# danisotelo/qm_door

Hardware: AMD Instinct MI355X
Metric: MPC+WBC cycles/sec (AlienGo+Z1, N=100) (higher is better)
Workload: dtype f64; 1 GPU; configs[1]: batch=256 MPC instances per GPU, horizon N=100, dt=0.015, trot, 1 SQP iteration + filter line search + 3-level WBC; batch_per_gpu=256, global_batch=256, horizon_nodes=100, gait=trot, seed=0, collective=none

## Files before the change

qm_door_amd/csrc/kernels/aux_kernels.h:

```cpp
#pragma once
#include "layout.h"
#include "lq_kernel.h"

namespace qmk {

__global__ void __launch_bounds__(64) input_weight_kernel(const ProblemR* P, const real* zeros, real* Rw) {
  __shared__ real J[12 * 12];
  __shared__ real RJ[12 * 12];
  const int lane = threadIdx.x;
  const ModelR& md = P->model;
  const int dd = lane < AD_DIRS ? lane : AD_DIRS - 1;
  const AdIn in{P->settings.initial_state, zeros, P->settings.initial_state, dd, 0.0_r};
  FlowOut<Du, Du3, Du3> f;
  BaseMotion2<Du, Du3> bm;
  centroidalSweep2<Du, Du3, Du3>(
      md, P->settings.gravity, in,
      [&](int c, Vec3<Du>, Vec3<Du3> v) {
        if (lane >= 3 && lane < 15) { const int j = lane - 3; J[(3 * c + 0) * 12 + j] = v.x.e; J[(3 * c + 1) * 12 + j] = v.y.e; J[(3 * c + 2) * 12 + j] = v.z.e; }
      },
      [&](Vec3<Du>, const Mat3<Du>&) { return Vec3<Du3>(); }, f, bm);
  __syncthreads();
  const real* Rt = P->settings.R_task;
  for (int e = lane; e < 144; e += 64) {
    const int i = e / 12, j = e % 12;
// ... 92 lines not shown
  constexpr int NB = 4;
  const real* tg = gridP + size_t(inst) * (Np + 1);
  const int K = Np + 1, last = K - 1;
  for (int k0 = wave * NB; k0 <= Nn; k0 += nw * NB) {
    real t[NB]; int lb[NB];
#pragma unroll
    for (int q = 0; q < NB; ++q) { t[q] = gridN[size_t(inst) * (Nn + 1) + min(k0 + q, Nn)]; lb[q] = 0; }
    for (int base = 0; base < K; base += 64) {
      const int i = base + lane;
      const real g = tg[i < K ? i : 0];
#pragma unroll
      for (int q = 0; q < NB; ++q) lb[q] += qmPopCount(qmBallot(i < K && g < t[q]));
    }
    real ta[NB], tb[NB];
#pragma unroll
    for (int q = 0; q < NB; ++q) { const int ic = max(0, min(lb[q] - 1, K - 2)); ta[q] = tg[ic]; tb[q] = tg[min(ic + 1, last)]; }
    int idx[NB]; real alpha[NB];
#pragma unroll
    for (int q = 0; q < NB; ++q) {
      const int interval = lb[q] - 1;
      const real len = tb[q] - ta[q];
      const real a = (len > 2.0_r * REAL_EPS) ? (tb[q] - t[q]) / len : 1.0_r;
      const bool before = interval < 0 || K <= 1, after = !before && interval >= last;
      idx[q] = before ? 0 : (after ? max(last - 1, 0) : interval);
      alpha[q] = before ? 1.0_r : (after ? 0.0_r : a);
    }
    const bool isX = lane < 30, isU = lane >= 32 && lane < 62;
    const int c = isX ? lane : (isU ? lane - 32 : 0);
    real l[NB], r[NB];
#pragma unroll
    for (int q = 0; q < NB; ++q) {
      const int iu0 = min(idx[q], Np - 1), iu1 = min(idx[q] + 1, Np - 1);
      const real* pl = isU ? Up + (size_t(inst) * Np + iu0) * 30 : Xp + (size_t(inst) * (Np + 1) + idx[q]) * 30;
      const real* pr = isU ? Up + (size_t(inst) * Np + iu1) * 30 : Xp + (size_t(inst) * (Np + 1) + min(idx[q] + 1, last)) * 30;
      l[q] = pl[c]; r[q] = pr[c];
    }
    const real x0v = (x0 && isX) ? x0[size_t(inst) * 30 + c] : 0.0_r;
#pragma unroll
    for (int q = 0; q < NB; ++q) { QM_KEEP(l[q]); QM_KEEP(r[q]); }
#pragma unroll
    for (int q = 0; q < NB; ++q) {
      const int k = k0 + q;
      const real v = alpha[q] * l[q] + (1.0_r - alpha[q]) * r[q];
      if (k <= Nn && isX) warmX[(size_t(inst) * (Nn + 1) + k) * 30 + c] = (k == 0 && x0) ? x0v : v;
      else if (k < Nn && isU) warmU[(size_t(inst) * Nn + k) * 30 + c] = v;
    }
  }
}

__global__ void __launch_bounds__(64) policy_eval_kernel(int batch, int N, const real* tgrid, const real* X, const real* U, const int* modes, const real* tEval,
                                                         real* xOut, real* uOut, int* modeOut) {
  const int inst = blockIdx.x, lane = threadIdx.x;
  if (inst >= batch) return;
  const real* tg = tgrid + size_t(inst) * (N + 1);
  const real t = tEval[inst];
  int idx; real alpha;
  timeSegmentWave(tg, N + 1, t, lane, idx, alpha);
  const int kMode = gridCountBelow(tg + 1, N, t, lane);
  if (lane < 30) {
    const real* xl = X + (size_t(inst) * (N + 1) + idx) * 30;
    xOut[size_t(inst) * 30 + lane] = alpha * xl[lane] + (1.0_r - alpha) * xl[30 + lane];
  } else if (lane >= 32 && lane < 62) {
    const int i = lane - 32, iu0 = min(idx, N - 1), iu1 = min(idx + 1, N - 1);
    const real* ul = U + (size_t(inst) * N + iu0) * 30; const real* ur = U + (size_t(inst) * N + iu1) * 30;
    uOut[size_t(inst) * 30 + i] = alpha * ul[i] + (1.0_r - alpha) * ur[i];
  } else if (lane == 63) {
    modeOut[inst] = modes[size_t(inst) * (N + 1) + kMode];
  }
}

}
```

qm_door_amd/csrc/kernels/linesearch_kernel.h:

```cpp
#pragma once
#include "layout.h"
#include "ls_lds.h"
#include "schedule_dev.h"
#include "sweep_dev.h"

namespace qmk {

struct LsArgs {
  const ProblemR* P;
  const real* Rw;
  int batch, N, K, lineSearch;
  const real* eeContact;
  const real* tgrid; const real* dtgrid; const int* nodePhase;
  const real* X; const real* U; const real* dX; const real* dU;
  const real* targetTimes; const real* targetStates;
  const int* schedNum; const real* schedTimes; const int* schedModes;
  const real* metrics;
  const real* instStats;
  const int* nodeMode;
  real* Xt; real* Ut;
  real* outT; real* outX; real* outU; int* outMode; real* outStats;
  int iteration;
  int trialInLds;
  int* done;
};

inline int lsThreads(int B, int N, int cus) { return (B > cus && N + 1 <= LS_MAX_THREADS / 2) ? LS_MAX_THREADS / 2 : LS_MAX_THREADS; }
struct LsLaunch { int threads, dynamicLdsBytes, trialInLds; };
inline LsLaunch lsLaunch(int B, int N, int cus) {
  const int threads = lsThreads(B, N, cus), bytes = lsTrialLdsBytes(N, threads);
  return LsLaunch{threads, bytes, bytes > 0};
}

struct DblIn {
  const real* x; const real* u; real dtS; const real* k1;
  __device__ __forceinline__ real hn(int i) const { return x[i] + dtS * k1[i]; }
  __device__ __forceinline__ real euler(int i) const { return x[9 + i] + dtS * k1[9 + i]; }
  __device__ __forceinline__ real q(int j) const { return x[12 + j] + dtS * u[12 + j]; }
  __device__ __forceinline__ real qd(int j) const { return u[12 + j]; }
  __device__ __forceinline__ Vec3<real> force(int c) const { return Vec3<real>(u[3 * c], u[3 * c + 1], u[3 * c + 2]); }
};

template <class WP> __device__ __attribute__((noinline)) void nodePerformance(const ModelR& md, const SettingsR& st, WP Qw, WP Rw, int weightStructure, const real* bc, const Schedule& sched, const real* tTimes, const real* tStates, const real* contact, int K, real t, real dt, int phase,
                                       bool terminal, const real* x, const real* u, const real* xnext, real& cost, real& dyn, real& eq, real* xnOut = nullptr) {
  QM_TICK_DECL;
  const int mode = sched.modes[phase];
  real eePosRef[3], eeQuatRef[4];
  eeReference(tTimes, tStates, K, t, eePosRef, eeQuatRef);
  real Ke = 0.0_r, fRef[3] = {0.0_r, 0.0_r, 0.0_r}, pEnv[3] = {0.0_r, 0.0_r, 0.0_r};
  if (contact && !terminal) { Ke = st.ee_contact_stiffness; eeContactReference(tTimes, contact, K, t, fRef, pEnv); }
  real k1[12];
#pragma unroll
  for (int i = 0; i < 12; ++i) k1[i] = 0.0_r;
  real c = 0.0_r;
  dyn = 0.0_r; eq = 0.0_r;
  real phi[12];
#pragma unroll 1
  for (int stage = 0; stage < (terminal ? 1 : 2); ++stage) {
    const DblIn in{x, u, stage ? dt : 0.0_r, k1};
    Feet<real> feet;
    real f[12];
    BaseMotion<real> bm;
    centroidalSweep<real>(
        md, st.gravity, in, [&](int cc, Vec3<real> r, Vec3<real> v) { feet.set(cc, r, v); },
        [&](Vec3<real> r, const Mat3<real>& R) {
          const real sdt = stage ? dt : 0.0_r;
          const Vec3<real> fe(-Ke * (x[6] + sdt * k1[6] + r.x - pEnv[0]), -Ke * (x[7] + sdt * k1[7] + r.y - pEnv[1]), -Ke * (x[8] + sdt * k1[8] + r.z - pEnv[2]));
          if (stage == 0) {
            const real muF = Ke != 0.0_r ? st.ee_force_mu : 0.0_r;
            c += 0.5_r * muF * ((fe.x - fRef[0]) * (fe.x - fRef[0]) + (fe.y - fRef[1]) * (fe.y - fRef[1]) + (fe.z - fRef[2]) * (fe.z - fRef[2]));
            real qee[4];
            matrixToQuaternion(R, qee);
            const Vec3<real> od = quaternionDistance(qee, eeQuatRef);
            const real muP = terminal ? st.ee_final_mu_position : st.ee_mu_position, muO = terminal ? st.ee_final_mu_orientation : st.ee_mu_orientation;
            const real hx = x[6] + r.x - eePosRef[0], hy = x[7] + r.y - eePosRef[1], hz = x[8] + r.z - eePosRef[2];
            c += 0.5_r * muP * (hx * hx + hy * hy + hz * hz) + 0.5_r * muO * (od.x * od.x + od.y * od.y + od.z * od.z);
          }
// ... 227 lines not shown
        const real al = tr ? alpha * st.alpha_decay : alpha;
        if (tr && al < st.alpha_min) break;
        real s0 = 0, s1 = 0, s2 = 0;
        const int nTrial = N + 1 < half ? N + 1 : half;
        for (int i = tr * half; i < tr * half + nTrial; ++i) { s0 += red[0][i]; s1 += red[1][i]; s2 += red[2][i]; }
        m1 = s0; v1 = sqrt(s1 + s2);
        bool ok;
        if (!a.lineSearch) { ok = true; type = 0; }
        else if (v1 > st.g_max) { ok = v1 < (1.0_r - st.gamma_c) * viol0; type = 1; }
        else if (v1 < st.g_min && viol0 < st.g_min && al * armijo < 0.0_r) { ok = m1 < merit0 + st.armijo_factor * al * armijo; type = 3; }
        else { ok = m1 < merit0 - st.gamma_c * viol0 || v1 < (1.0_r - st.gamma_c) * viol0; type = 2; }
        accAlpha = al;
        if (ok) acc = 1.0_r;
      }
      ctl[LS_MERIT1] = m1; ctl[LS_VIOL1] = v1; ctl[LS_ACCEPTED] = acc; ctl[LS_STEP_TYPE] = real(type); ctl[LS_ALPHA] = accAlpha;
    }
    __syncthreads();
    QM_LS_CLOCK(4);
    merit1 = ctl[LS_MERIT1]; viol1 = ctl[LS_VIOL1]; stepType = int(ctl[LS_STEP_TYPE]);
    accepted = ctl[LS_ACCEPTED] != 0.0_r;
    const real lastAlpha = ctl[LS_ALPHA];
    __syncthreads();
    if (accepted) { alpha = lastAlpha; break; }
    alpha = lastAlpha * st.alpha_decay;
    if (alpha < st.alpha_min) break;
  }
  if (!accepted) { alpha = 0.0_r; stepType = 4; merit1 = merit0; viol1 = viol0; }
  real* oX = a.outX + size_t(inst) * (N + 1) * 30; real* oU = a.outU + size_t(inst) * N * 30;
  axpyStrided(oX, X, dX, alpha, (N + 1) * 30, tid, nthr);
  axpyStrided(oU, U, dU, alpha, N * 30, tid, nthr);
  for (int k = tid; k <= N; k += nthr) { a.outT[size_t(inst) * (N + 1) + k] = tg[k]; a.outMode[size_t(inst) * (N + 1) + k] = a.nodeMode[size_t(inst) * (N + 1) + k]; }
  QM_LS_CLOCK(5);
  const real sx = sumSquaresStrided(dX, (N + 1) * 30, tid, nthr), su = sumSquaresStrided(dU, N * 30, tid, nthr);
  __syncthreads();
  red[0][tid] = sx; red[1][tid] = su;
  __syncthreads();
  if (tid == 0) {
    real s0 = 0, s1 = 0;
    for (int i = 0; i < nthr; ++i) { s0 += red[0][i]; s1 += red[1][i]; }
    int conv = 0;
    if (a.iteration + 1 >= st.sqp_iterations) conv = 1;
    else if (alpha < st.alpha_min) conv = 2;
    else if (fabs(merit1 - merit0) < st.cost_tol && viol1 < st.g_min) conv = 3;
    else if (alpha * sqrt(s0) < st.delta_tol && alpha * sqrt(s1) < st.delta_tol) conv = 4;
    if (ricStatus != 0.0_r && conv == 0) conv = 2;
    a.done[inst] = conv;
    if (a.outStats) {
      real* s = a.outStats + size_t(inst) * QMGPU_NSTATS;
      s[0] = merit0; s[1] = viol0; s[2] = merit1; s[3] = viol1; s[4] = alpha; s[5] = real(stepType); s[6] = armijo; s[7] = ricStatus;
      s[8] = real(a.iteration + 1); s[9] = real(conv);
    }
  }
  QM_LS_CLOCK(6);
}
#endif

}
```

qm_door_amd/csrc/kernels/mpc_pipeline.h:

```cpp
#pragma once
#include <vector>

#include "../host/host_error.h"
#include "aux_kernels.h"
#include "ddp_kernel.h"
#include "gpu_rt.h"
#include "layout.h"
#include "linesearch_kernel.h"
#include "lq_kernel.h"
#include "riccati_kernel.h"

namespace qmk {

struct MpcBuffers {
  ProblemR* dP = nullptr;
  real *dRw = nullptr, *dZeros = nullptr;
  real *dTgrid = nullptr, *dDtgrid = nullptr, *dX = nullptr, *dU = nullptr, *dStages = nullptr, *dAdRows = nullptr, *dMetrics = nullptr, *dGains = nullptr, *ddX = nullptr, *ddU = nullptr;
  real *dXt = nullptr, *dUt = nullptr, *dInstStats = nullptr, *dDebug = nullptr;
  int *dStageNc = nullptr, *dNodeMode = nullptr, *dNodePhase = nullptr, *dDone = nullptr;
  real *dDdpX = nullptr, *dDdpU = nullptr, *dDdpMerit = nullptr;
  int cus = 256;
  size_t maxBatch = 0, maxNodes = 0;
};

struct MpcIo {
  int batch, N, K, lineSearch;
  double dtD;
  const double *t0D, *timeGridD, *schedTimesD;
  const real *x0, *targetTimes, *targetStates;
  const int* schedNum; const real* schedTimes; const int* schedModes;
  const real *warmX, *warmU;
  real *outT, *outX, *outU; int* outMode; real* outStats;
  const real* eeContact;
  int algorithm;
};

template <class Alloc> inline void allocateMpcBuffers(MpcBuffers& m, size_t B, size_t N, Alloc&& alloc) {
  const size_t N1 = N + 1;
  m.maxBatch = B; m.maxNodes = N;
  auto R = [&](size_t n, bool scratch = true) { return static_cast<real*>(alloc(n, sizeof(real), scratch)); };
  auto I = [&](size_t n) { return static_cast<int*>(alloc(n, sizeof(int), true)); };
  m.dP = static_cast<ProblemR*>(alloc(1, sizeof(ProblemR), false));
  m.dRw = R(QM_RW_DOUBLES, false);
  m.dZeros = R(64, false);
  m.dTgrid = R(B * N1);
  m.dDtgrid = R(B * N1);
  m.dNodePhase = I(B * N1);
  m.dX = R(B * N1 * 30);
  m.dU = R(B * N * 30);
  m.dStages = R(B * N1 * STAGE_DOUBLES);
  m.dAdRows = R(B * N1 * AD_DOUBLES);
  m.dMetrics = R(B * N1 * NODE_METRICS);
  m.dGains = R(B * N * GAIN_DOUBLES);
  m.ddX = R(B * N1 * 30);
  m.ddU = R(B * N * 30);
  m.dXt = R(2 * B * N1 * 30);
  m.dUt = R(2 * B * N * 30);
  m.dInstStats = R(B * 4);
  m.dStageNc = I(B * N1);
  m.dNodeMode = I(B * N1);
  m.dDone = I(B);
  int dev = 0, cus = 0;
  if (hipGetDevice(&dev) == hipSuccess && hipDeviceGetAttribute(&cus, hipDeviceAttributeMultiprocessorCount, dev) == hipSuccess && cus > 0) m.cus = cus;
}

template <class Alloc> inline void ensureDdpBuffers(MpcBuffers& m, Alloc&& alloc) {
  if (m.dDdpX) return;
  const size_t B = m.maxBatch, N = m.maxNodes;
  m.dDdpX = static_cast<real*>(alloc(size_t(DDP_MAX_TRIALS) * B * (N + 1) * 30, sizeof(real), true));
  m.dDdpU = static_cast<real*>(alloc(size_t(DDP_MAX_TRIALS) * B * N * 30, sizeof(real), true));
  m.dDdpMerit = static_cast<real*>(alloc(size_t(DDP_MAX_TRIALS) * B * 2, sizeof(real), true));
}

inline hipError_t prepareMpcKernels() {
  const hipError_t e = QM_ALLOW_DYNAMIC_LDS(riccati_kernel<RICCATI_WAVES>, RICCATI_LDS_BYTES);
  return e != hipSuccess ? e : QM_ALLOW_DYNAMIC_LDS(linesearch_kernel, QM_CU_LDS_BYTES - LS_STATIC_LDS_BYTES);
}

struct MpcStaging {
  real *x0 = nullptr, *targetTimes = nullptr, *targetStates = nullptr, *schedTimes = nullptr, *warmX = nullptr, *warmU = nullptr, *eeContact = nullptr;
};

template <class In> inline MpcIo makeMpcIo(const qmgpu_mpc_args& a, double dt, const MpcStaging& st, In&& in, real* outT, real* outX, real* outU, real* outStats) {
  const size_t B = size_t(a.batch), N = size_t(a.num_nodes), N1 = N + 1, K = size_t(a.num_target_knots);
  MpcIo io{};
  io.batch = a.batch; io.N = a.num_nodes; io.K = a.num_target_knots; io.lineSearch = a.line_search;
  io.dtD = dt; io.t0D = a.t0; io.timeGridD = a.time_grid; io.schedTimesD = a.sched_event_times;
  io.x0 = in(a.x0, st.x0, B * 30);
  io.targetTimes = in(a.target_times, st.targetTimes, B * K);
  io.targetStates = in(a.target_states, st.targetStates, B * K * QMGPU_NTARGET);
  io.schedNum = a.sched_num_events;
  io.schedTimes = in(a.sched_event_times, st.schedTimes, B * QMGPU_MAX_EVENTS);
  io.schedModes = a.sched_modes;
  io.warmX = in(a.warm_x, st.warmX, B * N1 * 30);
  io.warmU = in(a.warm_u, st.warmU, B * N * 30);
  io.eeContact = in(a.ee_contact_ref, st.eeContact, B * K * 6);
  io.outT = outT; io.outX = outX; io.outU = outU; io.outMode = a.out_mode; io.outStats = outStats;
  io.algorithm = a.algorithm;
  return io;
}

enum TimingEvent { EV_START, EV_AD_NODE, EV_LQ_NODE, EV_RICCATI, EV_LINE_SEARCH, EV_WBC_START, EV_WBC_END, TIMING_EVENTS = EV_WBC_END + 1 };
inline void recordTiming(hipEvent_t* ev, TimingEvent which, hipStream_t s) { if (ev) (void)hipEventRecord(ev[which], s); }

inline void enqueueLqRiccati(hipStream_t s, const MpcBuffers& m, const MpcIo& io, real* debug, hipEvent_t* ev) {
  const int B = io.batch, N = io.N;
  LqArgs la{m.dP, m.dRw, B, N, io.K, m.dTgrid, m.dDtgrid, m.dNodePhase, m.dX, m.dU, io.targetTimes, io.targetStates, io.schedNum, io.schedTimes,
            io.schedModes, m.dZeros, m.dStages, m.dStageNc, m.dNodeMode, m.dMetrics, debug, m.dAdRows, m.dDone, io.eeContact};
  QM_LAUNCH(ad_node_kernel, adGridFor(B * (N + 1)), 64, s, la);
  recordTiming(ev, EV_AD_NODE, s);
  QM_LAUNCH(lq_node_kernel, B * (N + 1), 64, s, la);
  recordTiming(ev, EV_LQ_NODE, s);
  RiccatiArgs ra{B, N, m.dStages, m.dStageNc, m.dDtgrid, io.x0, m.dX, m.dGains, m.ddX, m.ddU, m.dInstStats, m.dDone};
  QM_LAUNCH_DYN(riccati_kernel<RICCATI_WAVES>, B, RICCATI_WAVES * 64, RICCATI_LDS_BYTES, s, ra);
  recordTiming(ev, EV_RICCATI, s);
}

inline void enqueueMpcKernels(hipStream_t s, const MpcBuffers& m, const MpcIo& io, int iterations, bool debugLq, hipEvent_t* ev) {
  const int B = io.batch, N = io.N;
  recordTiming(ev, EV_START, s);
  for (int it = 0; it < iterations; ++it) {
    InitArgs ia{m.dP, B, N, io.dtD, io.t0D, io.timeGridD, io.schedTimesD, io.x0, it == 0 ? io.warmX : io.outX, it == 0 ? io.warmU : io.outU, io.schedNum, io.schedModes,
                m.dTgrid, m.dDtgrid, m.dNodePhase, m.dX, m.dU, it, m.dDone};
    QM_LAUNCH(mpc_init_kernel, B, 128, s, ia);
    enqueueLqRiccati(s, m, io, debugLq ? m.dDebug : nullptr, ev);
    const LsLaunch shape = lsLaunch(B, N, m.cus);
    LsArgs ls{m.dP, m.dRw, B, N, io.K, io.lineSearch, io.eeContact, m.dTgrid, m.dDtgrid, m.dNodePhase, m.dX, m.dU, m.ddX, m.ddU, io.targetTimes, io.targetStates, io.schedNum,
              io.schedTimes, io.schedModes, m.dMetrics, m.dInstStats, m.dNodeMode, m.dXt, m.dUt, io.outT, io.outX, io.outU, io.outMode, io.outStats, it, shape.trialInLds, m.dDone};
    QM_LAUNCH_DYN(linesearch_kernel, B, shape.threads, shape.dynamicLdsBytes, s, ls);
    recordTiming(ev, EV_LINE_SEARCH, s);
  }
}

inline void enqueueDdpKernels(hipStream_t s, const MpcBuffers& m, const MpcIo& io, int trials, hipEvent_t* ev) {
  const int B = io.batch, N = io.N;
  recordTiming(ev, EV_START, s);
  InitArgs ia{m.dP, B, N, io.dtD, io.t0D, io.timeGridD, io.schedTimesD, io.x0, io.warmX, io.warmU, io.schedNum, io.schedModes, m.dTgrid, m.dDtgrid, m.dNodePhase, m.dX, m.dU, 0, m.dDone};
  QM_LAUNCH(mpc_init_kernel, B, 128, s, ia);
  DdpArgs ra{m.dP, m.dRw, B, N, io.K, 0, io.eeContact, m.dTgrid, m.dDtgrid, m.dNodePhase, io.x0, m.dX, m.dU, io.targetTimes, io.targetStates, io.schedNum, io.schedTimes, io.schedModes,
             m.dStages, m.dStageNc, m.dGains, m.dX, m.dU, m.dDdpMerit};
  if (!io.warmX) QM_LAUNCH(ddp_rollout_kernel, (B + 63) / 64, 64, s, ra);
  enqueueLqRiccati(s, m, io, nullptr, ev);
  ra.trials = trials; ra.Xout = m.dDdpX; ra.Uout = m.dDdpU;
  QM_LAUNCH(ddp_rollout_kernel, (B * trials + 63) / 64, 64, s, ra);
  DdpSelectArgs sa{m.dP, B, N, trials, m.dTgrid, m.dNodeMode, m.dX, m.dU, m.dMetrics, m.dInstStats, m.dDdpX, m.dDdpU, m.dDdpMerit, io.outT, io.outX, io.outU, io.outMode, io.outStats, m.dDone};
  QM_LAUNCH(ddp_select_kernel, B, 256, s, sa);
  recordTiming(ev, EV_LINE_SEARCH, s);
}

inline int ddpTrialCount(double minStep, double maxStep) {
  int n = 0;
  for (double a = maxStep; a >= minStep && n < DDP_MAX_TRIALS; a *= 0.5) ++n;
  return n > 0 ? n : 1;
}

template <class Alloc> inline void enqueueMpcSolve(hipStream_t s, MpcBuffers& m, const MpcIo& io, const qmgpu_settings& settings, bool debugLq, hipEvent_t* ev, Alloc&& alloc) {
  if (io.algorithm != QMGPU_ALG_SQP && io.algorithm != QMGPU_ALG_DDP) throw std::invalid_argument("unknown qmgpu_mpc_args::algorithm");
  if (io.algorithm == QMGPU_ALG_DDP) {
    ensureDdpBuffers(m, alloc);
    enqueueDdpKernels(s, m, io, ddpTrialCount(settings.ddp_min_step, settings.ddp_max_step), ev);
  } else {
    enqueueMpcKernels(s, m, io, settings.sqp_iterations > 1 ? settings.sqp_iterations : 1, debugLq, ev);
  }
  HIP_CHECK(hipGetLastError());
}

}
```

qm_door_amd/csrc/kernels/schedule_dev.h:

```cpp
#pragma once
#include "problem_r.h"
#include "contact_rows.h"
#include "gpu_rt.h"

namespace qmk {

struct Schedule {
  int numEvents;
  const real* eventTimes;
  const int* modes;
};

__device__ __forceinline__ int nodePhaseAt(const Schedule& s, real t) {
  int i = 0;
  while (i < s.numEvents && s.eventTimes[i] <= t) ++i;
  return i;
}

__device__ __forceinline__ void cubic(real t0, real p0, real v0, real t1, real p1, real v1, real t, real& pos, real& vel) {
  const real dt = t1 - t0, dp = p1 - p0, dv = v1 - v0;
  const real c1 = v0 * dt, c2 = -(3.0_r * v0 + dv) * dt + 3.0_r * dp, c3 = (2.0_r * v0 + dv) * dt - 2.0_r * dp;
  const real tn = (t - t0) / dt;
  pos = ((c3 * tn + c2) * tn + c1) * tn + p0;
  vel = ((3.0_r * c3 * tn + 2.0_r * c2) * tn + c1) / dt;
// ... 1 lines not shown

__device__ inline void swingReference(const SettingsR& st, const Schedule& s, int leg, real t, int phase, real& zpos, real& zvel) {
  const int numPhases = s.numEvents + 1;
  int startIdx = -1;
  for (int ip = phase - 1; ip >= 0; --ip) if (contactOf(s.modes[ip], leg)) { startIdx = ip; break; }
  int finalIdx = numPhases - 1;
  for (int ip = phase + 1; ip < numPhases; ++ip) if (contactOf(s.modes[ip], leg)) { finalIdx = ip - 1; break; }
  const real tStart = (startIdx >= 0) ? s.eventTimes[startIdx] : ((s.numEvents > 0 ? s.eventTimes[0] : t) - st.touchdown_after_horizon);
  const real tFinal = (finalIdx < numPhases - 1) ? s.eventTimes[finalIdx] : ((s.numEvents > 0 ? s.eventTimes[s.numEvents - 1] : t) + st.touchdown_after_horizon);
  const real scaling = fmin(1.0_r, (tFinal - tStart) / st.swing_time_scale);
  const real tMid = 0.5_r * (tStart + tFinal), midHeight = scaling * st.swing_height;
  if (t < tMid) cubic(tStart, 0.0_r, scaling * st.liftoff_velocity, tMid, midHeight, 0.0_r, t, zpos, zvel);
  else cubic(tMid, midHeight, 0.0_r, tFinal, 0.0_r, scaling * st.touchdown_velocity, t, zpos, zvel);
}

__device__ __forceinline__ void timeSegment(const real* times, int K, real t, int& index, real& alpha) {
  if (K <= 1) { index = 0; alpha = 1.0_r; return; }
  int lb = 0;
  while (lb < K && times[lb] < t) ++lb;
  const int interval = lb - 1, last = K - 1;
  if (interval < 0) { index = 0; alpha = 1.0_r; }
  else if (interval >= last) { index = max(last - 1, 0); alpha = 0.0_r; }
  else {
    const real len = times[interval + 1] - times[interval];
    index = interval;
    alpha = (len > 2.0_r * REAL_EPS) ? (times[interval + 1] - t) / len : 1.0_r;
  }
}

__device__ __forceinline__ int gridCountBelow(const real* times, int K, real t, int lane) {
  int lb = 0;
  for (int base = 0; base < K; base += 64) {
    const int i = base + lane;
    const bool below = i < K && times[i < K ? i : 0] < t;
    const unsigned long long m = qmBallot(below);
    lb += qmPopCount(m);
    if (m != ~0ull) break;
  }
  return lb;
}
__device__ __forceinline__ void timeSegmentWave(const real* times, int K, real t, int lane, int& index, real& alpha) {
  if (K <= 1) { index = 0; alpha = 1.0_r; return; }
  const int lb = gridCountBelow(times, K, t, lane);
  const int interval = lb - 1, last = K - 1;
  if (interval < 0) { index = 0; alpha = 1.0_r; }
  else if (interval >= last) { index = max(last - 1, 0); alpha = 0.0_r; }
  else {
    const real len = times[interval + 1] - times[interval];
    index = interval;
    alpha = (len > 2.0_r * REAL_EPS) ? (times[interval + 1] - t) / len : 1.0_r;
  }
}

__device__ inline void eeReference(const real* times, const real* states, int K, real t, real pos[3], real quat[4]) {
  int idx; real alpha;
  timeSegment(times, K, t, idx, alpha);
  const real* lhs = states + size_t(idx) * QMGPU_NTARGET;
  if (K <= 1) {
    for (int i = 0; i < 3; ++i) pos[i] = lhs[30 + i];
    for (int i = 0; i < 4; ++i) quat[i] = lhs[33 + i];
    return;
  }
  const real* rhs = lhs + QMGPU_NTARGET;
  for (int i = 0; i < 3; ++i) pos[i] = alpha * lhs[30 + i] + (1.0_r - alpha) * rhs[30 + i];
  const real tt = 1.0_r - alpha;
  const real* a = lhs + 33; const real* b = rhs + 33;
  const real d = a[0] * b[0] + a[1] * b[1] + a[2] * b[2] + a[3] * b[3];
  const real absD = fabs(d);
  real s0, s1;
  if (absD >= 1.0_r - REAL_EPS) { s0 = 1.0_r - tt; s1 = tt; }
  else { const real theta = acos(absD), sinTheta = sin(theta); s0 = sin((1.0_r - tt) * theta) / sinTheta; s1 = sin(tt * theta) / sinTheta; }
  if (d < 0) s1 = -s1;
  for (int i = 0; i < 4; ++i) quat[i] = s0 * a[i] + s1 * b[i];
}
__device__ inline void eeContactReference(const real* times, const real* contact, int K, real t, real fref[3], real env[3]) {
  int idx; real alpha;
  timeSegment(times, K, t, idx, alpha);
  const real* lhs = contact + size_t(idx) * 6;
  const real* rhs = K > 1 ? lhs + 6 : lhs;
  for (int i = 0; i < 3; ++i) { fref[i] = alpha * lhs[i] + (1.0_r - alpha) * rhs[i]; env[i] = alpha * lhs[3 + i] + (1.0_r - alpha) * rhs[3 + i]; }
}
__device__ __forceinline__ real xReference(const real* states, int K, int idx, real alpha, int i) {
  const real* lhs = states + size_t(idx) * QMGPU_NTARGET;
  if (K <= 1) return lhs[i];
  return alpha * lhs[i] + (1.0_r - alpha) * lhs[QMGPU_NTARGET + i];
}

struct Barrier {
  real mu, delta;
  __device__ __forceinline__ real value(real h) const { const real q = (h - 2.0_r * delta) / delta; return h > delta ? -mu * log(h) : mu * (-log(delta) + 0.5_r * q * q - 0.5_r); }
  __device__ __forceinline__ real d1(real h) const { return h > delta ? -mu / h : mu * ((h - 2.0_r * delta) / (delta * delta)); }
  __device__ __forceinline__ real d2(real h) const { return h > delta ? mu / (h * h) : mu / (delta * delta); }
  __device__ __forceinline__ void eval(real h, real logDelta, real& val, real& g, real& hs) const {
    if (h > delta) { const real r = 1.0_r / h; val = -mu * log(h); g = -mu * r; hs = mu * r * r; }
    else { const real q = (h - 2.0_r * delta) / delta; val = mu * (-logDelta + 0.5_r * q * q - 0.5_r); g = mu * ((h - 2.0_r * delta) / (delta * delta)); hs = mu / (delta * delta); }
  }
  __device__ __forceinline__ real valueL(real h, real logDelta) const {
    if (h > delta) return -mu * log(h);
    const real q = (h - 2.0_r * delta) / delta;
    return mu * (-logDelta + 0.5_r * q * q - 0.5_r);
  }
};

}
```

qm_door_amd/csrc/qmgpu_api.hip:

```cpp
#include <algorithm>
#include <cstdio>
#include <cstring>
#include <memory>
#include <string>
#include <vector>

#include "../../include/qmgpu.h"
#include "host/host_error.h"
#include "kernels/mpc_pipeline.h"
#include "kernels/feedback_kernel.h"
#include "kernels/value_kernel.h"
#include "kernels/dual_kernel.h"
#include "kernels/wbc_kernel.h"
#include "kernels/frontend_kernel.h"
#include "mpc32.h"

using namespace qmhost;
using namespace qmk;

struct DeviceGuard {
  int prev = -1;
  explicit DeviceGuard(int device, bool mayThrow = true) {
    if (hipGetDevice(&prev) != hipSuccess) prev = -1;
    if (prev == device) { prev = -1; return; }
// ... 185 lines not shown
    double v;
    if (e < nx) v = X[size_t(inst) * nx + e];
    else if (e < nx + nu) v = U[size_t(inst) * nu + (e - nx)];
    else if (e < nx + nu + QMGPU_NWBC_OUT) v = wbc[size_t(inst) * QMGPU_NWBC_OUT + (e - nx - nu)];
    else v = double(modes[size_t(inst) * (N + 1) + (e - nx - nu - QMGPU_NWBC_OUT)]);
    row[e] = v;
  }
}

#ifdef QM_RICCATI_TIMING
int qmgpu_debug_riccati_ticks(unsigned long long* out64, int reset) {
  if (hipDeviceSynchronize() != hipSuccess) return QMGPU_ERR_HIP;
  if (out64 && hipMemcpyFromSymbol(out64, HIP_SYMBOL(qmk::qmRiccatiTicks), sizeof(unsigned long long) * 2048) != hipSuccess) return QMGPU_ERR_HIP;
  if (reset) { static unsigned long long z[2048] = {}; if (hipMemcpyToSymbol(HIP_SYMBOL(qmk::qmRiccatiTicks), z, sizeof(z)) != hipSuccess) return QMGPU_ERR_HIP; }
  return QMGPU_OK;
}
int qmgpu_debug_ad_wg_clocks(unsigned long long* out64, int count) {
  if (hipDeviceSynchronize() != hipSuccess) return QMGPU_ERR_HIP;
  if (count > 2 * QM_AD_WG_CLOCKS) count = 2 * QM_AD_WG_CLOCKS;
  if (hipMemcpyFromSymbol(out64, HIP_SYMBOL(qmk::qmAdWgClock), sizeof(unsigned long long) * size_t(count)) != hipSuccess) return QMGPU_ERR_HIP;
  return QMGPU_OK;
}
#endif

int qmgpu_debug_poison(qmgpu_handle h) {
  return onHandle(h, [&]() {
    joinWbc(h);
    for (auto& sc : h->scratch) HIP_CHECK(hipMemsetAsync(sc.first, 0xFF, sc.second, h->stream));
    constexpr int kDoubles = QM_CU_LDS_BYTES / 8;
    HIP_CHECK(QM_ALLOW_DYNAMIC_LDS(lds_poison_kernel, kDoubles * 8));
    QM_LAUNCH_DYN(lds_poison_kernel, 4096, 256, kDoubles * 8, h->stream, kDoubles, static_cast<double*>(nullptr));
    HIP_CHECK(hipGetLastError());
  });
}

int qmgpu_enable_debug(qmgpu_handle h, int enable) {
  return onHandle(h, [&]() {
    if (enable && h->dtype != QMGPU_F64) throw std::invalid_argument("the per-node LQ dump exists in the fp64 path only");
    if (enable && !h->m.dDebug) h->m.dDebug = h->alloc<double>(size_t(h->maxBatch) * (h->maxNodes + 1) * DBG_DOUBLES);
    h->debugLq = enable != 0;
  });
}

static void checkMpcArgs(qmgpu_handle h, const qmgpu_mpc_args* a) {
  if (!a) throw std::invalid_argument("null argument");
  if (a->batch < 1 || a->num_nodes < 1 || a->num_target_knots < 1) throw std::invalid_argument("batch, num_nodes and num_target_knots must be positive");
  if (a->batch > h->maxBatch || a->num_nodes > h->maxNodes) throw CapacityError("batch / num_nodes exceed the capacity given to qmgpu_create");
  if (h->dtype == QMGPU_F32 && a->num_target_knots > QMGPU_F32_MAX_TARGET_KNOTS) throw CapacityError("an fp32 handle stages at most QMGPU_F32_MAX_TARGET_KNOTS target knots per instance");
  if (!a->x0 || !a->target_times || !a->target_states || !a->sched_num_events || !a->sched_event_times || !a->sched_modes) throw std::invalid_argument("missing MPC input pointer");
  if (!a->time_grid && !a->t0) throw std::invalid_argument("either t0 or time_grid is required");
  if (!a->out_t || !a->out_x || !a->out_u || !a->out_mode) throw std::invalid_argument("missing MPC output pointer");
}

static void enqueueMpc(qmgpu_handle h, const qmgpu_mpc_args* a) {
  const qmgpu_settings& settings = h->hostProblem.settings;
  hipEvent_t* ev = h->timing ? h->ev : nullptr;
  if (h->dtype == QMGPU_F32) {
    qmk32::enqueue(h->m32, h->stream, a, settings, ev, h->rawAlloc);
  } else {
    const MpcIo io = makeMpcIo(*a, settings.dt, MpcStaging{}, [](const double* src, double*, size_t) { return src; }, a->out_t, a->out_x, a->out_u, a->out_stats);
    enqueueMpcSolve(h->stream, h->m, io, settings, h->debugLq, ev, h->rawAlloc);
  }
  h->lastBatch = a->batch; h->lastN = a->num_nodes; h->lastAlgorithm = a->algorithm;
  h->lastDebugLq = h->dtype == QMGPU_F64 && a->algorithm == QMGPU_ALG_SQP && h->debugLq;
}

static void enqueueWbc(qmgpu_handle h, const qmgpu_wbc_args* w, hipStream_t stream) {
  if (!w || w->batch < 1) throw std::invalid_argument("bad WBC arguments");
  if (w->batch > h->maxBatch) throw CapacityError("WBC batch exceeds the capacity given to qmgpu_create");
  if (!w->state_desired || !w->input_desired || !w->rbd_measured || !w->mode || !w->period || !w->time || !w->input_last || !w->out) throw std::invalid_argument("missing WBC pointer");
  static_assert(sizeof(unsigned long long) == sizeof(uint64_t), "working-set words");
  WbcArgs wa{h->m.dP, w->batch, w->variant, w->state_desired, w->input_desired, w->rbd_measured, w->mode, w->period, w->time, w->input_last, w->out, w->out_status, w->ee_force,
             reinterpret_cast<unsigned long long*>(w->working_set)};
  QM_LAUNCH_DYN(wbc_kernel, w->batch, WBC_THREADS, WBC_LDS_BYTES, stream, wa);
  HIP_CHECK(hipGetLastError());
}

static void beginTiming(qmgpu_handle h) {
  if (h->timing) h->ev = h->ring[h->callCount % qmgpu_context::kRing];
}
static void finishTiming(qmgpu_handle h, bool mpc, bool wbc) {
  if (!h->timing) return;
  h->ringKind[h->callCount % qmgpu_context::kRing] = (mpc ? 1 : 0) | (wbc ? 2 : 0);
  ++h->callCount;
}
static void readTiming(qmgpu_handle h, long call, double* ms6) {
  hipEvent_t* ev = h->ring[call % qmgpu_context::kRing];
  const int kind = h->ringKind[call % qmgpu_context::kRing];
  const bool mpc = kind & 1, wbc = kind & 2;
  const TimingEvent first = mpc ? EV_START : EV_WBC_START, last = wbc ? EV_WBC_END : EV_LINE_SEARCH;
  HIP_CHECK(hipEventSynchronize(ev[last]));
  auto elapsed = [&](TimingEvent from, TimingEvent to) { float ms = 0.f; HIP_CHECK(hipEventElapsedTime(&ms, ev[from], ev[to])); return double(ms); };
  for (int i = 0; i < 6; ++i) ms6[i] = 0.0;
  if (mpc) for (int k = EV_AD_NODE; k <= EV_LINE_SEARCH; ++k) ms6[k - EV_AD_NODE] = elapsed(TimingEvent(k - 1), TimingEvent(k));
  if (wbc) ms6[4] = elapsed(EV_WBC_START, EV_WBC_END);
  ms6[5] = elapsed(first, last);
}

int qmgpu_mpc_solve_batch(qmgpu_handle h, const qmgpu_mpc_args* args) {
  return onHandle(h, [&]() { checkMpcArgs(h, args); beginTiming(h); enqueueMpc(h, args); finishTiming(h, true, false); });
}

int qmgpu_policy_eval_batch(qmgpu_handle h, int batch, int num_nodes, const double* t_grid, const double* X, const double* U, const int32_t* modes, const double* t_eval,
                            double* x_out, double* u_out, int32_t* mode_out) {
  if (!t_grid || !X || !U || !modes || !t_eval || !x_out || !u_out || !mode_out || batch < 1 || num_nodes < 1) return setError(QMGPU_ERR_INVALID_ARGUMENT, "bad arguments");
  return onHandle(h, [&]() {
    QM_LAUNCH(policy_eval_kernel, batch, 64, h->stream, batch, num_nodes, t_grid, X, U, modes, t_eval, x_out, u_out, mode_out);
    HIP_CHECK(hipGetLastError());
  });
}

static void checkLastSqpSolve(qmgpu_handle h, int batch, int num_nodes, const char* what) {
  const std::string w(what);
  if (h->dtype != QMGPU_F64) throw std::invalid_argument(w + " exists for QMGPU_F64 handles only");
  if (h->lastBatch < 1) throw std::invalid_argument(w + " needs a solve on this handle first");
  if (h->lastAlgorithm != QMGPU_ALG_SQP) throw std::invalid_argument(w + " exists for QMGPU_ALG_SQP solves only");
  if (batch != h->lastBatch || num_nodes != h->lastN) throw std::invalid_argument("batch / num_nodes differ from the last solve on this handle");
}

int qmgpu_mpc_feedback_batch(qmgpu_handle h, int batch, int num_nodes, const double* X, const double* U, double* K, double* uff, int32_t* status) {
  if (!X || !U || !K || !uff || batch < 1 || num_nodes < 1) return setError(QMGPU_ERR_INVALID_ARGUMENT, "bad feedback arguments");
  return onHandle(h, [&]() {
    checkLastSqpSolve(h, batch, num_nodes, "the feedback policy");
    static_assert(sizeof(int) == sizeof(int32_t), "status words");
    FeedbackArgs fa{batch, num_nodes, h->m.dStages, h->m.dGains, h->m.dInstStats, X, U, K, uff, status};
    QM_LAUNCH(feedback_gain_kernel, batch * (num_nodes + 1), 64, h->stream, fa);
    HIP_CHECK(hipGetLastError());
  });
}

int qmgpu_mpc_value_function_batch(qmgpu_handle h, int batch, int num_nodes, double* Sm, double* Sv, double* sv_lin, double* x_lin, int32_t* status) {
  if (!Sm || !Sv || batch < 1 || num_nodes < 1) return setError(QMGPU_ERR_INVALID_ARGUMENT, "bad value-function arguments");
  return onHandle(h, [&]() {
    checkLastSqpSolve(h, batch, num_nodes, "the value function");
    ValueArgs va{batch, num_nodes, h->m.dStages, h->m.dGains, h->m.dDtgrid, h->m.dInstStats, h->m.dX, Sm, Sv, sv_lin, x_lin, status};
    QM_LAUNCH_DYN(value_function_kernel, batch, VALUE_THREADS, VALUE_LDS_BYTES, h->stream, va);
    HIP_CHECK(hipGetLastError());
  });
}

int qmgpu_mpc_dual_batch(qmgpu_handle h, int batch, int num_nodes, double* costate, double* nu, int32_t* nc, int32_t* status) {
  if (!costate || batch < 1 || num_nodes < 1) return setError(QMGPU_ERR_INVALID_ARGUMENT, "bad dual-solution arguments");
  return onHandle(h, [&]() {
    checkLastSqpSolve(h, batch, num_nodes, "the dual solution");
    if (nu && !(h->lastDebugLq && h->m.dDebug)) throw std::invalid_argument("nu needs the LQ dump of the solve: call qmgpu_enable_debug(h, 1) before it");
    static_assert(sizeof(int) == sizeof(int32_t), "nc and status words");
    DualArgs da{batch, num_nodes, h->m.dStages, h->m.dGains, h->m.dDtgrid, h->m.dInstStats, h->m.ddX, h->m.ddU, nu ? h->m.dDebug : nullptr, h->m.dStageNc, costate, nu, nc, status};
    QM_LAUNCH_DYN(costate_kernel, batch, DUAL_THREADS, DUAL_LDS_BYTES, h->stream, da);
// ... 23 lines not shown

int qmgpu_frontend_batch(qmgpu_handle h, const qmgpu_frontend_args* a) {
  if (!a || a->batch < 1 || !a->rbd_measured || !a->time || !a->command_kind || !a->command || !a->last_ee_target || !a->x0 || !a->target_times || !a->target_states)
    return setError(QMGPU_ERR_INVALID_ARGUMENT, "bad front-end arguments");
  return onHandle(h, [&]() {
    FrontendArgs fa{h->m.dP, *a};
    QM_LAUNCH(frontend_kernel, (a->batch + 63) / 64, 64, h->stream, fa);
    HIP_CHECK(hipGetLastError());
  });
}

int qmgpu_gait_schedule_batch(qmgpu_handle h, int batch, const qmgpu_gait* templates, int num_templates, const int32_t* gait_index, const int32_t* prev_mode,
                              const double* t_phase0, const double* t_begin, const double* t_end, int32_t* sched_num_events, double* sched_event_times, int32_t* sched_modes, int32_t* status) {
  if (batch < 1 || !templates || num_templates < 1 || num_templates > 64 || !gait_index || !t_phase0 || !t_begin || !t_end || !sched_num_events || !sched_event_times || !sched_modes)
    return setError(QMGPU_ERR_INVALID_ARGUMENT, "bad gait schedule arguments");
  return onHandle(h, [&]() {
    if (!h->dGaits) h->dGaits = h->alloc<qmgpu_gait>(64, false);
    HIP_CHECK(hipMemcpyAsync(h->dGaits, templates, sizeof(qmgpu_gait) * num_templates, hipMemcpyHostToDevice, h->stream));
    HIP_CHECK(hipStreamSynchronize(h->stream));
    GaitArgs ga{batch, num_templates, h->dGaits, gait_index, prev_mode, h->hostProblem.settings.phase_transition_stance_time, t_phase0, t_begin, t_end, sched_num_events, sched_event_times, sched_modes, status};
    QM_LAUNCH(gait_schedule_kernel, (batch + 63) / 64, 64, h->stream, ga);
    HIP_CHECK(hipGetLastError());
  });
}

int qmgpu_wbc_solve_batch(qmgpu_handle h, const qmgpu_wbc_args* args) {
  return onHandle(h, [&]() {
    joinWbc(h);
    beginTiming(h);
    if (h->timing) HIP_CHECK(hipEventRecord(h->ev[EV_WBC_START], h->stream));
    enqueueWbc(h, args, h->stream);
    if (h->timing) HIP_CHECK(hipEventRecord(h->ev[EV_WBC_END], h->stream));
    finishTiming(h, false, true);
  });
}

int qmgpu_warm_start_batch(qmgpu_handle h, int batch, int prev_nodes, const double* prev_grid, const double* prev_X, const double* prev_U, int new_nodes,
                           const double* new_grid, const double* x0, double* warm_x, double* warm_u) {
  if (!prev_grid || !prev_X || !prev_U || !new_grid || !warm_x || !warm_u || batch < 1 || prev_nodes < 1 || new_nodes < 1)
    return setError(QMGPU_ERR_INVALID_ARGUMENT, "bad warm-start arguments");
  if (warm_x == prev_X || warm_u == prev_U) return setError(QMGPU_ERR_INVALID_ARGUMENT, "warm-start outputs must not alias the previous solution");
  return onHandle(h, [&]() {
    QM_LAUNCH(warm_start_kernel, batch, 256, h->stream, batch, prev_nodes, prev_grid, prev_X, prev_U, new_nodes, new_grid, x0, warm_x, warm_u);
    HIP_CHECK(hipGetLastError());
  });
}

int qmgpu_cycle_batch(qmgpu_handle h, const qmgpu_mpc_args* mpc, const double* t_eval, qmgpu_wbc_args* wbc) {
  if (!t_eval || !wbc) return setError(QMGPU_ERR_INVALID_ARGUMENT, "null argument");
  return onHandle(h, [&]() {
    checkMpcArgs(h, mpc);
    if (wbc->batch != mpc->batch) throw std::invalid_argument("MPC and WBC batch sizes differ");
    beginTiming(h);
    enqueueMpc(h, mpc);
    joinWbc(h);
    QM_LAUNCH(policy_eval_kernel, mpc->batch, 64, h->stream, mpc->batch, mpc->num_nodes, mpc->out_t, mpc->out_x, mpc->out_u, mpc->out_mode, t_eval, h->dPolX, h->dPolU,
              h->dPolMode);
    qmgpu_wbc_args w = *wbc;
    w.state_desired = h->dPolX; w.input_desired = h->dPolU; w.mode = h->dPolMode;
    hipStream_t ws = h->stream;
    if (h->overlap) {
      HIP_CHECK(hipEventRecord(h->evPolicy, h->stream));
      HIP_CHECK(hipStreamWaitEvent(h->wbcStream, h->evPolicy, 0));
      ws = h->wbcStream;
    }
    if (h->timing) HIP_CHECK(hipEventRecord(h->ev[EV_WBC_START], ws));
    enqueueWbc(h, &w, ws);
    if (h->timing) HIP_CHECK(hipEventRecord(h->ev[EV_WBC_END], ws));
    if (h->overlap) { HIP_CHECK(hipEventRecord(h->evWbc, ws)); h->wbcPending = true; }
    finishTiming(h, true, true);
  });
}

int qmgpu_debug_get_lq(qmgpu_handle h, int instance, int node, double* A, double* B, double* b, double* Q, double* R, double* q, double* r, double* C, double* D, double* e,
                       int32_t* nc) {
  return onHandle(h, [&]() {
    if (!h->debugLq || !h->m.dDebug) throw std::invalid_argument("call qmgpu_enable_debug(h, 1) before the solve");
    if (instance < 0 || instance >= h->lastBatch || node < 0 || node > h->lastN) throw std::invalid_argument("instance / node out of range");
    HIP_CHECK(hipStreamSynchronize(h->stream));
    std::vector<double> rec(DBG_DOUBLES);
    const size_t idx = size_t(instance) * (h->lastN + 1) + node;
    HIP_CHECK(hipMemcpy(rec.data(), h->m.dDebug + idx * DBG_DOUBLES, DBG_DOUBLES * sizeof(double), hipMemcpyDeviceToHost));
    int ncv = 0;
    HIP_CHECK(hipMemcpy(&ncv, h->m.dStageNc + idx, sizeof(int), hipMemcpyDeviceToHost));
    auto cp = [&](double* dst, int off, int n) { if (dst) std::memcpy(dst, rec.data() + off, n * sizeof(double)); };
    cp(A, DBG_A, 900); cp(B, DBG_B, 900); cp(b, DBG_b, 30); cp(Q, DBG_Q, 900); cp(R, DBG_R, 900); cp(q, DBG_q, 30); cp(r, DBG_r, 30);
    cp(C, DBG_C, 16 * 30); cp(D, DBG_D, 16 * 30); cp(e, DBG_e, 16);
    if (nc) *nc = ncv;
  });
}

int qmgpu_last_kernel_ms(qmgpu_handle h, double* ms6) {
  if (!ms6) return setError(QMGPU_ERR_INVALID_ARGUMENT, "null argument");
  return onHandle(h, [&]() {
    if (!h->timing || h->callCount == 0) throw std::invalid_argument("no timed call recorded (qmgpu_enable_timing)");
    readTiming(h, h->callCount - 1, ms6);
  });
}

int qmgpu_kernel_ms_mean(qmgpu_handle h, int last_calls, double* ms6) {
  if (!ms6 || last_calls < 1) return setError(QMGPU_ERR_INVALID_ARGUMENT, "bad argument");
  return onHandle(h, [&]() {
    if (!h->timing || h->callCount == 0) throw std::invalid_argument("no timed call recorded (qmgpu_enable_timing)");
    const long n = std::min<long>(std::min<long>(last_calls, h->callCount), qmgpu_context::kRing);
    double acc[6] = {0, 0, 0, 0, 0, 0};
    for (long c = h->callCount - n; c < h->callCount; ++c) { double m[6]; readTiming(h, c, m); for (int i = 0; i < 6; ++i) acc[i] += m[i]; }
    for (int i = 0; i < 6; ++i) ms6[i] = acc[i] / double(n);
  });
}

int qmgpu_pack_results(qmgpu_handle h, int batch, int num_nodes, const double* X, const double* U, const double* wbc_out, const int32_t* modes, double* packed) {
  if (!X || !U || !wbc_out || !modes || !packed || batch < 1 || num_nodes < 1) return setError(QMGPU_ERR_INVALID_ARGUMENT, "bad arguments");
  return onHandle(h, [&]() {
    QM_LAUNCH(pack_results_kernel, batch, 256, h->stream, batch, num_nodes, X, U, wbc_out, modes, packed);
    HIP_CHECK(hipGetLastError());
  });
}

int qmgpu_kernel_ms_history(qmgpu_handle h, int last_calls, double* ms6_per_call) {
  if (!ms6_per_call || last_calls < 1) return setError(QMGPU_ERR_INVALID_ARGUMENT, "bad argument");
  return onHandle(h, [&]() {
    if (!h->timing || h->callCount == 0) throw std::invalid_argument("no timed call recorded (qmgpu_enable_timing)");
    if (last_calls > h->callCount || last_calls > qmgpu_context::kRing) throw std::invalid_argument("more calls asked for than the event ring holds");
// ... 6 lines not shown
```

Before: 155,700 cycles/s.

## Fold policy evaluation into line-search kernel and relax WBC stream join

Moves the policy interpolation (state/input/mode at t_eval) into the tail of the line-search kernel, run by its last wave in the f64 SQP path. This removes a separate policy_eval kernel launch. The host-side joinWbc is replaced by a stream wait on the previous WBC event, placed just before the first line search, so the MPC's LQ and Riccati stages can overlap the previous cycle's WBC. Timing bookkeeping is adjusted so the WBC interval is measured from the line-search end event.

```diff
diff --git a/qm_door_amd/csrc/kernels/aux_kernels.h b/qm_door_amd/csrc/kernels/aux_kernels.h
--- a/qm_door_amd/csrc/kernels/aux_kernels.h
+++ b/qm_door_amd/csrc/kernels/aux_kernels.h
@@ -168,21 +168,8 @@
                                                          real* xOut, real* uOut, int* modeOut) {
   const int inst = blockIdx.x, lane = threadIdx.x;
   if (inst >= batch) return;
-  const real* tg = tgrid + size_t(inst) * (N + 1);
-  const real t = tEval[inst];
-  int idx; real alpha;
-  timeSegmentWave(tg, N + 1, t, lane, idx, alpha);
-  const int kMode = gridCountBelow(tg + 1, N, t, lane);
-  if (lane < 30) {
-    const real* xl = X + (size_t(inst) * (N + 1) + idx) * 30;
-    xOut[size_t(inst) * 30 + lane] = alpha * xl[lane] + (1.0_r - alpha) * xl[30 + lane];
-  } else if (lane >= 32 && lane < 62) {
-    const int i = lane - 32, iu0 = min(idx, N - 1), iu1 = min(idx + 1, N - 1);
-    const real* ul = U + (size_t(inst) * N + iu0) * 30; const real* ur = U + (size_t(inst) * N + iu1) * 30;
-    uOut[size_t(inst) * 30 + i] = alpha * ul[i] + (1.0_r - alpha) * ur[i];
-  } else if (lane == 63) {
-    modeOut[inst] = modes[size_t(inst) * (N + 1) + kMode];
-  }
+  policyEvalWave(N, tgrid + size_t(inst) * (N + 1), X + size_t(inst) * (N + 1) * 30, U + size_t(inst) * N * 30, modes + size_t(inst) * (N + 1), tEval[inst], lane,
+                 xOut + size_t(inst) * 30, uOut + size_t(inst) * 30, modeOut + inst);
 }
 
 }
diff --git a/qm_door_amd/csrc/kernels/linesearch_kernel.h b/qm_door_amd/csrc/kernels/linesearch_kernel.h
--- a/qm_door_amd/csrc/kernels/linesearch_kernel.h
+++ b/qm_door_amd/csrc/kernels/linesearch_kernel.h
@@ -23,6 +23,7 @@
   int iteration;
   int trialInLds;
   int* done;
+  const double* tEval; double* polX; double* polU; int* polMode;
 };
 
 inline int lsThreads(int B, int N, int cus) { return (B > cus && N + 1 <= LS_MAX_THREADS / 2) ? LS_MAX_THREADS / 2 : LS_MAX_THREADS; }
@@ -356,7 +357,12 @@
     }
   }
   QM_LS_CLOCK(6);
-}
+#ifdef QM_REAL_IS_DOUBLE
+  if (a.tEval && tid >= nthr - 64)
+    policyEvalWave(N, a.outT + size_t(inst) * (N + 1), oX, oU, a.outMode + size_t(inst) * (N + 1), a.tEval[inst], tid - (nthr - 64), a.polX + size_t(inst) * 30,
+                   a.polU + size_t(inst) * 30, a.polMode + inst);
 #endif
-
-}
+}
+#endif
+
+}
diff --git a/qm_door_amd/csrc/kernels/mpc_pipeline.h b/qm_door_amd/csrc/kernels/mpc_pipeline.h
--- a/qm_door_amd/csrc/kernels/mpc_pipeline.h
+++ b/qm_door_amd/csrc/kernels/mpc_pipeline.h
@@ -8,6 +8,7 @@
 #include "layout.h"
 #include "linesearch_kernel.h"
 #include "lq_kernel.h"
+#include "policy_fold.h"
 #include "riccati_kernel.h"
 
 namespace qmk {
@@ -33,6 +34,7 @@
   real *outT, *outX, *outU; int* outMode; real* outStats;
   const real* eeContact;
   int algorithm;
+  qmhost::PolicyFold fold;
 };
 
 template <class Alloc> inline void allocateMpcBuffers(MpcBuffers& m, size_t B, size_t N, Alloc&& alloc) {
@@ -81,7 +83,8 @@
   real *x0 = nullptr, *targetTimes = nullptr, *targetStates = nullptr, *schedTimes = nullptr, *warmX = nullptr, *warmU = nullptr, *eeContact = nullptr;
 };
 
-template <class In> inline MpcIo makeMpcIo(const qmgpu_mpc_args& a, double dt, const MpcStaging& st, In&& in, real* outT, real* outX, real* outU, real* outStats) {
+template <class In> inline MpcIo makeMpcIo(const qmgpu_mpc_args& a, double dt, const MpcStaging& st, In&& in, real* outT, real* outX, real* outU, real* outStats,
+                                            const qmhost::PolicyFold& fold = {}) {
   const size_t B = size_t(a.batch), N = size_t(a.num_nodes), N1 = N + 1, K = size_t(a.num_target_knots);
   MpcIo io{};
   io.batch = a.batch; io.N = a.num_nodes; io.K = a.num_target_knots; io.lineSearch = a.line_search;
@@ -97,6 +100,7 @@
   io.eeContact = in(a.ee_contact_ref, st.eeContact, B * K * 6);
   io.outT = outT; io.outX = outX; io.outU = outU; io.outMode = a.out_mode; io.outStats = outStats;
   io.algorithm = a.algorithm;
+  io.fold = fold;
   return io;
 }
 
@@ -125,8 +129,11 @@
     QM_LAUNCH(mpc_init_kernel, B, 128, s, ia);
     enqueueLqRiccati(s, m, io, debugLq ? m.dDebug : nullptr, ev);
     const LsLaunch shape = lsLaunch(B, N, m.cus);
+    const qmhost::PolicyFold& pf = io.fold;
+    if (it == 0 && pf.tEval && pf.overwriteAfter) HIP_CHECK(hipStreamWaitEvent(s, pf.overwriteAfter, 0));
     LsArgs ls{m.dP, m.dRw, B, N, io.K, io.lineSearch, io.eeContact, m.dTgrid, m.dDtgrid, m.dNodePhase, m.dX, m.dU, m.ddX, m.ddU, io.targetTimes, io.targetStates, io.schedNum,
-              io.schedTimes, io.schedModes, m.dMetrics, m.dInstStats, m.dNodeMode, m.dXt, m.dUt, io.outT, io.outX, io.outU, io.outMode, io.outStats, it, shape.trialInLds, m.dDone};
+              io.schedTimes, io.schedModes, m.dMetrics, m.dInstStats, m.dNodeMode, m.dXt, m.dUt, io.outT, io.outX, io.outU, io.outMode, io.outStats, it, shape.trialInLds, m.dDone,
+              pf.tEval, pf.x, pf.u, pf.mode};
     QM_LAUNCH_DYN(linesearch_kernel, B, shape.threads, shape.dynamicLdsBytes, s, ls);
     recordTiming(ev, EV_LINE_SEARCH, s);
   }
diff --git a/qm_door_amd/csrc/kernels/policy_fold.h b/qm_door_amd/csrc/kernels/policy_fold.h
--- /dev/null
+++ b/qm_door_amd/csrc/kernels/policy_fold.h
@@ -0,0 +1,19 @@
+#pragma once
+#ifdef QMGPU_HOST_EMULATION
+#include "gpu_rt.h"
+#else
+#include <hip/hip_runtime_api.h>
+#endif
+
+#include <cstdint>
+
+namespace qmhost {
+
+struct PolicyFold {
+  const double* tEval = nullptr;
+  double *x = nullptr, *u = nullptr;
+  int32_t* mode = nullptr;
+  hipEvent_t overwriteAfter = nullptr;
+};
+
+}
diff --git a/qm_door_amd/csrc/kernels/schedule_dev.h b/qm_door_amd/csrc/kernels/schedule_dev.h
--- a/qm_door_amd/csrc/kernels/schedule_dev.h
+++ b/qm_door_amd/csrc/kernels/schedule_dev.h
@@ -77,6 +77,22 @@
   }
 }
 
+__device__ __forceinline__ void policyEvalWave(int N, const real* tg, const real* X, const real* U, const int* modes, real t, int lane, real* xOut, real* uOut, int* modeOut) {
+  int idx; real alpha;
+  timeSegmentWave(tg, N + 1, t, lane, idx, alpha);
+  const int kMode = gridCountBelow(tg + 1, N, t, lane);
+  if (lane < 30) {
+    const real* xl = X + size_t(idx) * 30;
+    xOut[lane] = alpha * xl[lane] + (1.0_r - alpha) * xl[30 + lane];
+  } else if (lane >= 32 && lane < 62) {
+    const int i = lane - 32, iu0 = min(idx, N - 1), iu1 = min(idx + 1, N - 1);
+    const real* ul = U + size_t(iu0) * 30; const real* ur = U + size_t(iu1) * 30;
+    uOut[i] = alpha * ul[i] + (1.0_r - alpha) * ur[i];
+  } else if (lane == 63) {
+    *modeOut = modes[kMode];
+  }
+}
+
 __device__ inline void eeReference(const real* times, const real* states, int K, real t, real pos[3], real quat[4]) {
   int idx; real alpha;
   timeSegment(times, K, t, idx, alpha);
diff --git a/qm_door_amd/csrc/qmgpu_api.hip b/qm_door_amd/csrc/qmgpu_api.hip
--- a/qm_door_amd/csrc/qmgpu_api.hip
+++ b/qm_door_amd/csrc/qmgpu_api.hip
@@ -261,13 +261,13 @@
   if (!a->out_t || !a->out_x || !a->out_u || !a->out_mode) throw std::invalid_argument("missing MPC output pointer");
 }
 
-static void enqueueMpc(qmgpu_handle h, const qmgpu_mpc_args* a) {
+static void enqueueMpc(qmgpu_handle h, const qmgpu_mpc_args* a, const PolicyFold& fold = {}) {
   const qmgpu_settings& settings = h->hostProblem.settings;
   hipEvent_t* ev = h->timing ? h->ev : nullptr;
   if (h->dtype == QMGPU_F32) {
     qmk32::enqueue(h->m32, h->stream, a, settings, ev, h->rawAlloc);
   } else {
-    const MpcIo io = makeMpcIo(*a, settings.dt, MpcStaging{}, [](const double* src, double*, size_t) { return src; }, a->out_t, a->out_x, a->out_u, a->out_stats);
+    const MpcIo io = makeMpcIo(*a, settings.dt, MpcStaging{}, [](const double* src, double*, size_t) { return src; }, a->out_t, a->out_x, a->out_u, a->out_stats, fold);
     enqueueMpcSolve(h->stream, h->m, io, settings, h->debugLq, ev, h->rawAlloc);
   }
   h->lastBatch = a->batch; h->lastN = a->num_nodes; h->lastAlgorithm = a->algorithm;
@@ -288,9 +288,9 @@
 static void beginTiming(qmgpu_handle h) {
   if (h->timing) h->ev = h->ring[h->callCount % qmgpu_context::kRing];
 }
-static void finishTiming(qmgpu_handle h, bool mpc, bool wbc) {
+static void finishTiming(qmgpu_handle h, bool mpc, bool wbc, bool wbcFromLineSearch = false) {
   if (!h->timing) return;
-  h->ringKind[h->callCount % qmgpu_context::kRing] = (mpc ? 1 : 0) | (wbc ? 2 : 0);
+  h->ringKind[h->callCount % qmgpu_context::kRing] = (mpc ? 1 : 0) | (wbc ? 2 : 0) | (wbcFromLineSearch ? 4 : 0);
   ++h->callCount;
 }
 static void readTiming(qmgpu_handle h, long call, double* ms6) {
@@ -302,7 +302,7 @@
   auto elapsed = [&](TimingEvent from, TimingEvent to) { float ms = 0.f; HIP_CHECK(hipEventElapsedTime(&ms, ev[from], ev[to])); return double(ms); };
   for (int i = 0; i < 6; ++i) ms6[i] = 0.0;
   if (mpc) for (int k = EV_AD_NODE; k <= EV_LINE_SEARCH; ++k) ms6[k - EV_AD_NODE] = elapsed(TimingEvent(k - 1), TimingEvent(k));
-  if (wbc) ms6[4] = elapsed(EV_WBC_START, EV_WBC_END);
+  if (wbc) ms6[4] = elapsed((kind & 4) ? EV_LINE_SEARCH : EV_WBC_START, EV_WBC_END);
   ms6[5] = elapsed(first, last);
 }
 
@@ -432,23 +432,30 @@
     checkMpcArgs(h, mpc);
     if (wbc->batch != mpc->batch) throw std::invalid_argument("MPC and WBC batch sizes differ");
     beginTiming(h);
-    enqueueMpc(h, mpc);
-    joinWbc(h);
-    QM_LAUNCH(policy_eval_kernel, mpc->batch, 64, h->stream, mpc->batch, mpc->num_nodes, mpc->out_t, mpc->out_x, mpc->out_u, mpc->out_mode, t_eval, h->dPolX, h->dPolU,
-              h->dPolMode);
+    const bool folded = mpc->algorithm == QMGPU_ALG_SQP && h->dtype == QMGPU_F64;
+    if (folded) {
+      enqueueMpc(h, mpc, PolicyFold{t_eval, h->dPolX, h->dPolU, h->dPolMode, h->wbcPending ? h->evWbc : nullptr});
+      h->wbcPending = false;
+    } else {
+      enqueueMpc(h, mpc);
+      joinWbc(h);
+      QM_LAUNCH(policy_eval_kernel, mpc->batch, 64, h->stream, mpc->batch, mpc->num_nodes, mpc->out_t, mpc->out_x, mpc->out_u, mpc->out_mode, t_eval, h->dPolX, h->dPolU,
+                h->dPolMode);
+    }
     qmgpu_wbc_args w = *wbc;
     w.state_desired = h->dPolX; w.input_desired = h->dPolU; w.mode = h->dPolMode;
     hipStream_t ws = h->stream;
+    const bool startIsLineSearch = h->timing && folded;
     if (h->overlap) {
-      HIP_CHECK(hipEventRecord(h->evPolicy, h->stream));
-      HIP_CHECK(hipStreamWaitEvent(h->wbcStream, h->evPolicy, 0));
+      hipEvent_t handOff = startIsLineSearch ? h->ev[EV_LINE_SEARCH] : (h->timing ? h->ev[EV_WBC_START] : h->evPolicy);
+      if (!startIsLineSearch) HIP_CHECK(hipEventRecord(handOff, h->stream));
+      HIP_CHECK(hipStreamWaitEvent(h->wbcStream, handOff, 0));
       ws = h->wbcStream;
-    }
-    if (h->timing) HIP_CHECK(hipEventRecord(h->ev[EV_WBC_START], ws));
+    } else if (h->timing && !startIsLineSearch) HIP_CHECK(hipEventRecord(h->ev[EV_WBC_START], ws));
     enqueueWbc(h, &w, ws);
     if (h->timing) HIP_CHECK(hipEventRecord(h->ev[EV_WBC_END], ws));
     if (h->overlap) { HIP_CHECK(hipEventRecord(h->evWbc, ws)); h->wbcPending = true; }
-    finishTiming(h, true, true);
+    finishTiming(h, true, true, startIsLineSearch);
   });
 }
 
```

Measured after the change: 156,900 cycles/s, median of 6. About the same (+0.7%).
